# phd3/presto-1

Measured on AMD Instinct MI355X. Metric: probe_rows_per_sec, higher is better.
Workload: dtype int64+f64

## Files before the change

presto-1_amd/csrc/agg.h:

```cpp
#pragma once
#include <cstdlib>

#include "common.h"

namespace tgpu {

constexpr int kLimbs = 68;
constexpr int kMaxAggs = 16;
constexpr int64_t kOrdChainMaxGroups = 65536, kOrdChainMinRows = 256;
constexpr int64_t kOrdHandoffRows = 4096;
inline int64_t ord_chain_max_groups() { const char *e = getenv("TGPU_ORD_CHAIN_MAX_GROUPS"); return e ? atoll(e) : kOrdChainMaxGroups; }

class GroupedAccumulators {
public:
    GroupedAccumulators(Context *ctx, std::vector<tgpu_agg_spec> specs, int32_t step);

    void add_input(const int32_t *gids, int64_t n, const DevicePage &page, int64_t group_count, bool gids_ascending = false);
    void add_intermediate(const int32_t *gids, int64_t n, const DevicePage &page, int64_t group_count, bool gids_ascending = false);
    void evaluate(int64_t group_count, std::vector<DeviceColumn> &out);
    struct DeviceState {
        int32_t function;
        long long *counts;
        long long *limbs;
        unsigned int *special;
        unsigned long long *i128;
        double *dsum;
    };
    void reserve(int64_t groups) { ensure(groups > 0 ? groups : 1); }
    bool begin_ordered(const int32_t *gids, int64_t n, int64_t groups, int64_t lowcard_max_groups, BufferPtr &keys, BufferPtr &rows);
    BufferPtr group_stretches(const unsigned int *keys, int64_t n, int64_t ids);
    void set_allow_ordered(bool on) { allow_ordered_ = on; }
    void set_force_ordered(bool on) { force_ordered_ = on; }
    void set_combine_ordered(bool on) { combine_ordered_ = on; }
    bool force_ordered() const { return force_ordered_ && allow_ordered_; }
    bool ordered() const { return mode_ == Mode::ORDERED; }
    static constexpr int64_t kModePrefixRows = 65536;
    bool decided() const { return mode_ != Mode::UNDECIDED; }
    void decide(int64_t groups_in_prefix, int64_t lowcard_max_groups = 0);
    static int64_t groups_among(Context *ctx, const int32_t *gids, const uint8_t *gids8, int64_t m);
    DeviceState device_state(int k) const;
    struct FoldScratch {
        unsigned long long *partials;
        int32_t stride;
        unsigned long long *pending;
    };
    FoldScratch fold_scratch(int64_t blocks, int64_t group_capacity);
    void flush_fold();
    void resolve_pending(int64_t blocks, bool commit);
    struct HostStates {
        int64_t groups = 0;
        struct Agg {
            std::vector<long long> counts, limbs;
            std::vector<unsigned int> special;
            std::vector<unsigned long long> i128;
            std::vector<double> dsum;
        };
        std::vector<Agg> aggs;
        int64_t bytes() const;
    };
    HostStates dump(int64_t groups);
    void merge(const int32_t *gids, const HostStates &run, int64_t live_groups);
    const std::vector<tgpu_agg_spec> specs() const;
    int output_channel_count() const;
    int intermediate_channel_count() const;
    int64_t estimated_size() const;

private:
    struct State {
        tgpu_agg_spec spec;
        BufferPtr counts;
        BufferPtr limbs;
        BufferPtr special;
        BufferPtr i128;
        BufferPtr dsum;
        int64_t cap = 0;
    };
    enum class Mode { UNDECIDED, EXACT, ORDERED };
    void ensure(int64_t groups);
    void decide_mode(int64_t groups, int64_t lowcard_max_groups);
    void sort_rows_by_group(const int32_t *gids, int64_t n, int64_t groups, BufferPtr &keys, BufferPtr &rows, bool gids_ascending = false);
    Mode mode_ = Mode::UNDECIDED;
    bool allow_ordered_ = false, force_ordered_ = false;
    Context *ctx_;
    std::vector<State> states_;
    int32_t step_;
    BufferPtr error_;
    BufferPtr fold_partials_, fold_pending_;
    bool combine_ordered_ = false;
    int64_t fold_rows_ = 0, fold_stride_ = 0;
    bool fold_dirty_ = false;
};

}
```

presto-1_amd/csrc/agg.hip:

```cpp
#include "agg.h"
#include "kernels.h"
#include "device_agg.h"

#include <rocprim/rocprim.hpp>

#include <algorithm>
#include <cstdlib>

namespace tgpu {

namespace {

constexpr int kBlock = 256;

struct AggView {
    int32_t function;
    int32_t pad;
    const void *input;
    const uint8_t *input_nulls;
    const uint8_t *mask;
    const uint8_t *mask_nulls;
    const void *input2;
    const uint8_t *input2_nulls;
    long long *counts;
    long long *limbs;
    unsigned int *special;
    unsigned long long *i128;
    double *dsum;
};

struct AggArgs {
    int32_t n_aggs;
    int32_t pad;
    AggView a[kMaxAggs];
};

#define kulisch_add tg_kulisch_add
#define i128_add tg_i128_add

template <bool INTERMEDIATE>
__global__ void __launch_bounds__(kBlock) agg_accumulate_kernel(AggArgs args, const int32_t *__restrict__ gids, int64_t n)
{
    for (int64_t r = (int64_t)blockIdx.x * kBlock + threadIdx.x; r < n; r += (int64_t)gridDim.x * kBlock) {
        const int64_t g = gids ? gids[r] : 0;
        if (g < 0) continue;
        for (int k = 0; k < args.n_aggs; k++) {
            const AggView &a = args.a[k];
            if (INTERMEDIATE) {
                const long long cnt = ((const long long *)a.input)[r];
                if (a.function == TGPU_AGG_COUNT_ALL || a.function == TGPU_AGG_COUNT_COLUMN) {
                    if (cnt) atomicAdd((unsigned long long *)&a.counts[g], (unsigned long long)cnt);
                    continue;
                }
                if (cnt == 0) continue;
                atomicAdd((unsigned long long *)&a.counts[g], (unsigned long long)cnt);
                if (a.function == TGPU_AGG_SUM_BIGINT) i128_add(&a.i128[g * 2], ((const long long *)a.input2)[r]);
                else if (tg_is_minmax(a.function)) tg_minmax_update(&a.i128[g * 2], tg_minmax_encode(a.function, ((const unsigned long long *)a.input2)[r]));
                else kulisch_add(&a.limbs[g * kLimbs], &a.special[g], ((const double *)a.input2)[r]);
                continue;
            }
            if (a.mask && ((a.mask_nulls && a.mask_nulls[r]) || !a.mask[r])) continue;
            if (a.function == TGPU_AGG_COUNT_ALL) {
                atomicAdd((unsigned long long *)&a.counts[g], 1ULL);
                continue;
            }
            if (a.input_nulls && a.input_nulls[r]) continue;
            atomicAdd((unsigned long long *)&a.counts[g], 1ULL);
            switch (a.function) {
            case TGPU_AGG_SUM_BIGINT: i128_add(&a.i128[g * 2], ((const long long *)a.input)[r]); break;
            case TGPU_AGG_MIN_BIGINT:
            case TGPU_AGG_MAX_BIGINT:
            case TGPU_AGG_MIN_DOUBLE:
            case TGPU_AGG_MAX_DOUBLE: tg_minmax_update(&a.i128[g * 2], tg_minmax_encode(a.function, ((const unsigned long long *)a.input)[r])); break;
            case TGPU_AGG_SUM_DOUBLE:
            case TGPU_AGG_AVG_DOUBLE: kulisch_add(&a.limbs[g * kLimbs], &a.special[g], ((const double *)a.input)[r]); break;
            case TGPU_AGG_AVG_BIGINT: kulisch_add(&a.limbs[g * kLimbs], &a.special[g], (double)((const long long *)a.input)[r]); break;
            default: break;
            }
        }
    }
}


__global__ void __launch_bounds__(kBlock) ordered_keys_kernel(const int32_t *__restrict__ gids, int64_t n, unsigned int *__restrict__ keys, int *__restrict__ rows,
                                                               unsigned int *__restrict__ unsorted)
{
    bool bad = false;
    for (int64_t r = (int64_t)blockIdx.x * kBlock + threadIdx.x; r < n; r += (int64_t)gridDim.x * kBlock) {
        const int32_t g = gids[r];
        keys[r] = (unsigned int)(g + 1);
        rows[r] = (int)r;
        bad = bad || (r > 0 && gids[r - 1] > g);
    }
    if (unsorted && __any(bad) && (threadIdx.x & 63) == 0) *unsorted = 1u;
}

__global__ void __launch_bounds__(kBlock) ordered_stretches_kernel(const unsigned int *__restrict__ keys, int64_t n, int *__restrict__ stretches)
{
    for (int64_t i = (int64_t)blockIdx.x * kBlock + threadIdx.x; i < n; i += (int64_t)gridDim.x * kBlock) {
        const unsigned int k = keys[i];
        if (k == 0) continue;
        if (i == 0 || keys[i - 1] != k) stretches[(size_t)(k - 1) * 2] = (int)i;
        if (i == n - 1 || keys[i + 1] != k) stretches[(size_t)(k - 1) * 2 + 1] = (int)(i + 1);
    }
}

template <bool INTERMEDIATE>
__global__ void __launch_bounds__(kBlock) agg_ordered_kernel(AggArgs args, const unsigned int *__restrict__ keys, const int *__restrict__ rows, int64_t n,
                                                              unsigned int *error, int64_t handoff, long long *list, unsigned int *list_count)
{
    for (int64_t i = (int64_t)blockIdx.x * kBlock + threadIdx.x; i < n; i += (int64_t)gridDim.x * kBlock) {
        const unsigned int key = keys[i];
        if (key == 0 || (i > 0 && keys[i - 1] == key)) continue;
        const int64_t g = (int64_t)key - 1;
        const int64_t stop = handoff > 0 ? (i + handoff < n ? i + handoff : n) : n;
        if (handoff > 0 && stop < n && keys[stop] == key) {
            const unsigned int at = atomicAdd(list_count, 1u);
            list[(size_t)at * 2] = g;
            list[(size_t)at * 2 + 1] = stop;
        }
#pragma unroll
        for (int k = 0; k < kMaxAggs; k++) {
            if (k >= args.n_aggs) break;
            const AggView &a = args.a[k];
            long long cnt = 0;
            double s = a.dsum ? a.dsum[g] : 0.0;
            __int128 big = 0;
            unsigned long long best = 0;
            for (int64_t j = i; j < stop && keys[j] == key; j++) {
                const int64_t r = rows[j];
                if (INTERMEDIATE) {
                    const long long c = ((const long long *)a.input)[r];
                    if (c == 0) continue;
                    cnt += c;
                    if (a.function == TGPU_AGG_SUM_BIGINT) big += ((const long long *)a.input2)[r];
                    else if (tg_is_minmax(a.function)) {
                        const unsigned long long c_ = tg_minmax_encode(a.function, ((const unsigned long long *)a.input2)[r]);
                        best = c_ > best ? c_ : best;
                    }
                    else if (a.function != TGPU_AGG_COUNT_ALL && a.function != TGPU_AGG_COUNT_COLUMN) s += ((const double *)a.input2)[r];
                    continue;
                }
                if (a.mask && ((a.mask_nulls && a.mask_nulls[r]) || !a.mask[r])) continue;
                if (a.function != TGPU_AGG_COUNT_ALL && a.input_nulls && a.input_nulls[r]) continue;
                cnt++;
                switch (a.function) {
                case TGPU_AGG_SUM_BIGINT: big += ((const long long *)a.input)[r]; break;
                case TGPU_AGG_MIN_BIGINT:
                case TGPU_AGG_MAX_BIGINT:
                case TGPU_AGG_MIN_DOUBLE:
                case TGPU_AGG_MAX_DOUBLE: {
                    const unsigned long long c_ = tg_minmax_encode(a.function, ((const unsigned long long *)a.input)[r]);
                    best = c_ > best ? c_ : best;
                    break;
                }
                case TGPU_AGG_SUM_DOUBLE:
                case TGPU_AGG_AVG_DOUBLE: s += ((const double *)a.input)[r]; break;
                case TGPU_AGG_AVG_BIGINT: s += (double)((const long long *)a.input)[r]; break;
                default: break;
                }
            }
            if (cnt) a.counts[g] += cnt;
            if (a.dsum) a.dsum[g] = s;
            if (best) tg_minmax_update(&a.i128[g * 2], best);
            if (a.i128 && big != 0) {
                const unsigned __int128 cur = ((unsigned __int128)a.i128[g * 2 + 1] << 64) | a.i128[g * 2];
                const unsigned __int128 nxt = cur + (unsigned __int128)big;
                a.i128[g * 2] = (unsigned long long)nxt;
                a.i128[g * 2 + 1] = (unsigned long long)(nxt >> 64);
            }
        }
    }
    (void)error;
}

struct OrdChainPlan {
    int32_t slot[kMaxAggs];
};

__device__ inline long long wave_sum_i64(long long v)
{
#pragma unroll
    for (int d = 32; d >= 1; d >>= 1) v += __shfl_xor(v, d, 64);
    return v;
}

__device__ inline void ordered_chain_group(const AggArgs &args, const OrdChainPlan &plan, const int *__restrict__ rows, int64_t g, long long s, long long e, double *vals,
                                           unsigned long long *cnt_lds, unsigned long long *lo_lds, long long *hi_lds)
{
    const int wave = threadIdx.x >> 6, lane = threadIdx.x & 63;
    if (threadIdx.x < kMaxAggs) {
        cnt_lds[threadIdx.x] = 0;
        lo_lds[threadIdx.x] = 0;
        hi_lds[threadIdx.x] = 0;
    }
    double *sum = nullptr;
    if (wave == 0) {
        __builtin_amdgcn_s_setprio(3);
#pragma unroll
        for (int k = 0; k < kMaxAggs; k++)
            if (k < args.n_aggs && plan.slot[k] == lane) sum = args.a[k].dsum;
    }
    double os = sum ? sum[g] : 0.0;
    __syncthreads();
    const long long tiles = (e - s + TG_ORD_TILE - 1) / TG_ORD_TILE;
    const int r = (wave - 1) * 64 + lane;
    long long row_next = (wave > 0 && s + r < e) ? rows[s + r] : 0;
    for (long long t = 0; t <= tiles; t++) {
        if (wave > 0 && t < tiles) {
            const long long j = s + t * TG_ORD_TILE + r;
            const long long row = row_next;
            if (j + TG_ORD_TILE < e) row_next = rows[j + TG_ORD_TILE];
            double *out = vals + (t & 1) * (TG_ORD_MAX_DOUBLES * TG_ORD_STRIDE) + r;
            const bool live = j < e;
#pragma unroll
            for (int k = 0; k < kMaxAggs; k++) {
                if (k >= args.n_aggs) break;
                const AggView &a = args.a[k];
                bool take = live;
                if (take && a.mask && ((a.mask_nulls && a.mask_nulls[row]) || !a.mask[row])) take = false;
                if (take && a.function != TGPU_AGG_COUNT_ALL && a.input_nulls && a.input_nulls[row]) take = false;
                const unsigned long long taken = __ballot(take);
                if (lane == 0 && taken) atomicAdd(&cnt_lds[k], (unsigned long long)__popcll(taken));
                if (a.function == TGPU_AGG_SUM_BIGINT) {
                    const long long v = take ? ((const long long *)a.input)[row] : 0;
                    const long long lo = wave_sum_i64((long long)(unsigned int)v), hi = wave_sum_i64(v >> 32);
                    if (lane == 0 && taken) {
                        atomicAdd(&lo_lds[k], (unsigned long long)lo);
                        atomicAdd((unsigned long long *)&hi_lds[k], (unsigned long long)hi);
                    }
                }
                else if (tg_is_minmax(a.function)) {
                    if (take) tg_minmax_update(&a.i128[g * 2], tg_minmax_encode(a.function, ((const unsigned long long *)a.input)[row]));
                }
                else if (plan.slot[k] >= 0 && live) {
                    double x = -0.0;
                    if (take) x = a.function == TGPU_AGG_AVG_BIGINT ? (double)((const long long *)a.input)[row] : ((const double *)a.input)[row];
                    out[plan.slot[k] * TG_ORD_STRIDE] = x;
                }
            }
        }
        else if (wave == 0 && t > 0 && sum) {
            const long long left = e - (s + (t - 1) * TG_ORD_TILE);
            os = tg_chain_add_tile(vals + ((t - 1) & 1) * (TG_ORD_MAX_DOUBLES * TG_ORD_STRIDE) + lane * TG_ORD_STRIDE, left < TG_ORD_TILE ? (int)left : TG_ORD_TILE, os);
        }
        __syncthreads();
    }
    if (sum) sum[g] = os;
    if (threadIdx.x == 64) {
#pragma unroll
        for (int k = 0; k < kMaxAggs; k++) {
            if (k >= args.n_aggs) break;
            const AggView &a = args.a[k];
            if (cnt_lds[k]) a.counts[g] += (long long)cnt_lds[k];
            if (a.function == TGPU_AGG_SUM_BIGINT && a.i128) {
                const __int128 big = (__int128)hi_lds[k] * ((__int128)1 << 32) + (__int128)lo_lds[k];
                const unsigned __int128 cur = ((unsigned __int128)a.i128[g * 2 + 1] << 64) | a.i128[g * 2];
                const unsigned __int128 nxt = cur + (unsigned __int128)big;
                a.i128[g * 2] = (unsigned long long)nxt;
                a.i128[g * 2 + 1] = (unsigned long long)(nxt >> 64);
            }
        }
    }
    __syncthreads();
}

__global__ void __launch_bounds__(TG_ORD_WAVES * 64) agg_ordered_chain_kernel(AggArgs args, OrdChainPlan plan, const int *__restrict__ stretches,
                                                                               const unsigned int *__restrict__ keys, const int *__restrict__ rows, int64_t n,
                                                                               const long long *__restrict__ list, const unsigned int *__restrict__ list_count)
{
    __shared__ __attribute__((aligned(16))) double vals[2 * TG_ORD_MAX_DOUBLES * TG_ORD_STRIDE];
    __shared__ unsigned long long cnt_lds[kMaxAggs], lo_lds[kMaxAggs];
    __shared__ long long hi_lds[kMaxAggs];
    if (stretches) {
        const long long s = stretches[(size_t)blockIdx.x * 2], e = stretches[(size_t)blockIdx.x * 2 + 1];
        if (e > s) ordered_chain_group(args, plan, rows, blockIdx.x, s, e, vals, cnt_lds, lo_lds, hi_lds);
        return;
    }
    const unsigned int count = *list_count;
    for (unsigned int b = blockIdx.x; b < count; b += gridDim.x) {
        const long long g = list[(size_t)b * 2], s = list[(size_t)b * 2 + 1];
        long long lo = s, hi = n;
        while (lo < hi) { const long long mid = (lo + hi) >> 1; if (keys[mid] <= (unsigned int)(g + 1)) lo = mid + 1; else hi = mid; }
        if (lo > s) ordered_chain_group(args, plan, rows, g, s, lo, vals, cnt_lds, lo_lds, hi_lds);
    }
}

using LowCardPlan = TgLowCardPlan;

struct LowCardStates {
    TgAggState st[kMaxAggs];
};

__global__ void __launch_bounds__(kBlock) agg_lowcard_kernel(AggArgs args, LowCardStates states, LowCardPlan plan, const int32_t *__restrict__ gids, int64_t n,
                                                              TgFoldScratch fold)
{
    extern __shared__ __attribute__((aligned(16))) unsigned char lds[];
    tg_lc_zero(lds, plan);
    for (int64_t r = (int64_t)blockIdx.x * kBlock + threadIdx.x; r < n; r += (int64_t)gridDim.x * kBlock) {
        const int g = gids ? gids[r] : 0;
        if (g < 0) continue;
        double *hi_base = tg_lc_hi(lds, plan, g), *lo_base = tg_lc_lo(lds, plan, g);
        unsigned int *cnt_base = tg_lc_cnt(lds, plan, g);
        for (int k = 0; k < args.n_aggs; k++) {
            const AggView &a = args.a[k];
            if (a.mask && ((a.mask_nulls && a.mask_nulls[r]) || !a.mask[r])) continue;
            if (a.function != TGPU_AGG_COUNT_ALL && a.input_nulls && a.input_nulls[r]) continue;
            cnt_base[plan.cnt_slot[k] * kBlock + threadIdx.x] += 1u;
            if (tg_is_minmax(a.function)) {
                tg_minmax_update(&a.i128[(size_t)g * 2], tg_minmax_encode(a.function, ((const unsigned long long *)a.input)[r]));
                continue;
            }
            const int w = plan.wide_slot[k];
            if (w < 0) continue;
            if (a.function == TGPU_AGG_SUM_BIGINT) {
                tg_lc_add_bigint(hi_base, lo_base, w, ((const long long *)a.input)[r]);
                continue;
            }
            const double v = a.function == TGPU_AGG_AVG_BIGINT ? (double)((const long long *)a.input)[r] : ((const double *)a.input)[r];
            if (!(fabs(v) <= 1.7976931348623157e308)) {
                tg_flag_special(&a.special[g], v);
                continue;
            }
            const double r = tg_lc_add_double(hi_base, lo_base, w, v);
            if (r != 0.0) tg_kulisch_add(&a.limbs[(size_t)g * kLimbs], &a.special[g], r);
        }
    }
    tg_lc_fold(lds, plan, states.st, fold);
}

__global__ void __launch_bounds__(kBlock) agg_fold_flush_kernel(TgFoldScratch fs, int rows, int n_aggs, LowCardStates states)
{
    tg_fold_flush(fs, rows, n_aggs, states.st);
}

struct KulischWindow {
    int top;
    unsigned int w0, w1, w2;
    bool sticky;
    unsigned int p1, p2;
    bool below;
    __device__ void init() { top = -1; w0 = w1 = w2 = 0; sticky = false; p1 = p2 = 0; below = false; }
    __device__ void push(int i, unsigned int digit)
    {
        if (digit) { top = i; w0 = digit; w1 = p1; w2 = p2; sticky = below; }
        below = below || p2 != 0;
        p2 = p1;
        p1 = digit;
    }
};

__device__ double kulisch_round(const long long *limbs, unsigned int special)
{
    if (special) {
        if ((special & 1u) || ((special & 2u) && (special & 4u))) return __longlong_as_double(0x7ff8000000000000LL);
        return (special & 2u) ? __longlong_as_double(0x7ff0000000000000LL) : __longlong_as_double((long long)0xfff0000000000000ULL);
    }
    KulischWindow pos, negw;
    pos.init();
    negw.init();
    long long carry = 0;
    unsigned int negc = 1;
    for (int i = 0; i < kLimbs; i++) {
        const long long v = limbs[i] + carry;
        const unsigned int digit = (unsigned int)(v & 0xffffffffLL);
        carry = v >> 32;
        pos.push(i, digit);
        const unsigned int nd = ~digit + negc;
        negc = (negc && digit == 0) ? 1u : 0u;
        negw.push(i, nd);
    }
    const bool neg = carry < 0;
    const KulischWindow &w = neg ? negw : pos;
    if (w.top < 0) return 0.0;
    const int hb = 31 - __clz((int)w.w0);
    const int t = w.top * 32 + hb;
    unsigned long long bits;
    if (t <= 52) {
        bits = w.top == 1 ? (((unsigned long long)w.w0 << 32) | w.w1) : (unsigned long long)w.w0;
    }
    else {
        const unsigned __int128 win = ((unsigned __int128)w.w0 << 64) | ((unsigned __int128)w.w1 << 32) | (unsigned __int128)w.w2;
        const int gpos = 64 + hb - 53;
        unsigned long long mant = (unsigned long long)(win >> (gpos + 1));
        const bool guard = (unsigned long long)(win >> gpos) & 1ULL;
        bool sticky = w.sticky || (win & (((unsigned __int128)1 << gpos) - 1)) != 0;
        long long e = (long long)t - 51;
        if (guard && (sticky || (mant & 1ULL))) {
            mant++;
            if (mant >> 53) { mant >>= 1; e++; }
        }
        if (e >= 2047) bits = 0x7ff0000000000000ULL;
        else bits = ((unsigned long long)e << 52) | (mant & 0xfffffffffffffULL);
    }
    if (neg) bits |= 1ULL << 63;
    return __longlong_as_double((long long)bits);
}

struct EvalView {
    int32_t function;
    int32_t partial;
    const long long *counts;
    const long long *limbs;
    const unsigned int *special;
    const unsigned long long *i128;
    const double *dsum;
    void *out0;
    uint8_t *out0_nulls;
    void *out1;
};
struct EvalArgs {
    int32_t n_aggs;
    int32_t pad;
    EvalView a[kMaxAggs];
};

__global__ void __launch_bounds__(kBlock) agg_evaluate_kernel(EvalArgs args, int64_t groups, unsigned int *error)
{
    const int64_t total = groups * args.n_aggs;
    for (int64_t i = (int64_t)blockIdx.x * kBlock + threadIdx.x; i < total; i += (int64_t)gridDim.x * kBlock) {
        const int k = (int)(i % args.n_aggs);
        const int64_t g = i / args.n_aggs;
        const EvalView &a = args.a[k];
        const long long cnt = a.counts[g];
        if (a.function == TGPU_AGG_COUNT_ALL || a.function == TGPU_AGG_COUNT_COLUMN) {
            ((long long *)a.out0)[g] = cnt;
            continue;
        }
        double dsum = 0.0;
        long long lsum = 0;
        if (tg_is_minmax(a.function)) lsum = (long long)tg_minmax_decode(a.function, a.i128[g * 2]);
        else if (a.function == TGPU_AGG_SUM_BIGINT) {
            const unsigned long long lo = a.i128[g * 2], hi = a.i128[g * 2 + 1];
            lsum = (long long)lo;
            const unsigned long long expect_hi = lsum < 0 ? ~0ULL : 0ULL;
            if (hi != expect_hi) atomicOr(error, 1u);
        }
// ... 235 lines not shown
        const HostStates::Agg &r = run.aggs[k];
        MergeArgs::A &a = args.a[k];
        a.function = st.spec.function;
        a.counts = st.counts->as<long long>();
        a.limbs = st.limbs ? st.limbs->as<long long>() : nullptr;
        a.special = st.special ? st.special->as<unsigned int>() : nullptr;
        a.i128 = st.i128 ? st.i128->as<unsigned long long>() : nullptr;
        a.dsum = st.dsum ? st.dsum->as<double>() : nullptr;
        a.r_counts = (const long long *)up(r.counts.data(), r.counts.size() * 8);
        a.r_limbs = (const long long *)up(r.limbs.data(), r.limbs.size() * 8);
        a.r_special = (const unsigned int *)up(r.special.data(), r.special.size() * 4);
        a.r_i128 = (const unsigned long long *)up(r.i128.data(), r.i128.size() * 8);
        a.r_dsum = (const double *)up(r.dsum.data(), r.dsum.size() * 8);
    }
    ctx_->sync();
    ProfileScope ps(ctx_, "agg_merge_states");
    agg_merge_states_kernel<<<grid_for(ctx_, run.groups * kLimbs), kBlock, 0, ctx_->stream()>>>(args, gids, run.groups);
    check_launch("agg_merge_states");
    ctx_->sync();
}

GroupedAccumulators::DeviceState GroupedAccumulators::device_state(int k) const
{
    const State &st = states_[(size_t)k];
    DeviceState d;
    d.function = st.spec.function;
    d.counts = st.counts ? st.counts->as<long long>() : nullptr;
    d.limbs = st.limbs ? st.limbs->as<long long>() : nullptr;
    d.special = st.special ? st.special->as<unsigned int>() : nullptr;
    d.i128 = st.i128 ? st.i128->as<unsigned long long>() : nullptr;
    d.dsum = st.dsum ? st.dsum->as<double>() : nullptr;
    return d;
}

const std::vector<tgpu_agg_spec> GroupedAccumulators::specs() const
{
    std::vector<tgpu_agg_spec> v;
    for (auto &s : states_) v.push_back(s.spec);
    return v;
}

int GroupedAccumulators::output_channel_count() const
{
    return step_ == TGPU_STEP_PARTIAL ? intermediate_channel_count() : (int)states_.size();
}

int GroupedAccumulators::intermediate_channel_count() const
{
    int n = 0;
    for (auto &s : states_) n += is_count(s.spec.function) ? 1 : 2;
    return n;
}

int64_t GroupedAccumulators::estimated_size() const
{
    int64_t s = 0;
    for (auto &st : states_) {
        s += st.cap * 8;
        if (st.limbs) s += st.cap * (kLimbs * 8 + 4);
        if (st.dsum) s += st.cap * 8;
        if (st.i128) s += st.cap * 16;
    }
    return s;
}

void GroupedAccumulators::ensure(int64_t groups)
{
    ZeroList zeros{};
    for (auto &st : states_) {
        if (groups <= st.cap) continue;
        int64_t cap = st.cap ? st.cap : 256;
        while (cap < groups) cap <<= 1;
        st.counts = grow(ctx_, st.counts, st.cap, cap, 8, zeros);
        if (is_double_state(st.spec.function)) {
            if (mode_ == Mode::ORDERED) st.dsum = grow(ctx_, st.dsum, st.cap, cap, 8, zeros);
            else {
                st.limbs = grow(ctx_, st.limbs, st.cap * kLimbs, cap * kLimbs, 8, zeros);
                st.special = grow(ctx_, st.special, st.cap, cap, 4, zeros);
            }
        }
        if (is_bigint_state(st.spec.function)) st.i128 = grow(ctx_, st.i128, st.cap * 2, cap * 2, 8, zeros);
        st.cap = cap;
    }
    if (zeros.n) {
        unsigned long long most = 0;
        for (int i = 0; i < zeros.n; i++) most = std::max(most, zeros.words[i]);
        multi_zero_kernel<<<grid_for(ctx_, (int64_t)most), kBlock, 0, ctx_->stream()>>>(zeros);
        check_launch("multi_zero");
    }
}

static void check_channel(const DevicePage &page, int ch, int32_t want_type, const char *what)
{
    TG_CHECK_ARG(ch >= 0 && ch < (int)page.cols.size(), std::string(what) + ": channel out of range");
    if (want_type) TG_CHECK_ARG(page.cols[ch].type == want_type, std::string(what) + ": unexpected channel type " + type_name(page.cols[ch].type));
}

static int64_t lowcard_bytes_per_group(const std::vector<tgpu_agg_spec> &specs)
{
    int64_t wide = 0;
    for (auto &s : specs) wide += (is_count(s.function) || is_minmax(s.function)) ? 0 : 1;
    return wide * 2 * kBlock * 8 + (int64_t)specs.size() * kBlock * 4;
}

void GroupedAccumulators::decide_mode(int64_t groups, int64_t lowcard_max_groups)
{
    if (mode_ != Mode::UNDECIDED) return;
    const bool many = groups > lowcard_max_groups || force_ordered_;
    mode_ = (allow_ordered_ && many && getenv("TGPU_DISABLE_ORDERED") == nullptr) ? Mode::ORDERED : Mode::EXACT;
}

void GroupedAccumulators::decide(int64_t groups_in_prefix, int64_t lowcard_max_groups)
{
    if (lowcard_max_groups <= 0) lowcard_max_groups = (160 * 1024) / std::max<int64_t>(lowcard_bytes_per_group(specs()), 1);
    decide_mode(groups_in_prefix > 0 ? groups_in_prefix : 1, lowcard_max_groups);
}

static __global__ void __launch_bounds__(kBlock) max_gid_kernel(const int32_t *__restrict__ gids, const uint8_t *__restrict__ gids8, int64_t m, int *out)
{
    int best = -1;
    for (int64_t i = (int64_t)blockIdx.x * kBlock + threadIdx.x; i < m; i += (int64_t)gridDim.x * kBlock) {
        const int g = gids8 ? (int)gids8[i] - 1 : gids[i];
        best = g > best ? g : best;
    }
#pragma unroll
    for (int d = 32; d >= 1; d >>= 1) {
        const int o = __shfl_down(best, d, 64);
        best = o > best ? o : best;
    }
    if ((threadIdx.x & 63) == 0 && best >= 0) atomicMax(out, best);
}

int64_t GroupedAccumulators::groups_among(Context *ctx, const int32_t *gids, const uint8_t *gids8, int64_t m)
{
    if (m <= 0 || (!gids && !gids8)) return 0;
    BufferPtr out = ctx->alloc(4);
    HIP_CHECK(hipMemsetAsync(out->ptr(), 0xff, 4, ctx->stream()));
    max_gid_kernel<<<(int)std::min<int64_t>(ceil_div(m, kBlock), 64), kBlock, 0, ctx->stream()>>>(gids, gids8, m, out->as<int>());
    check_launch("max_gid");
    return (int64_t)ctx->read_scalar(out->as<int>()) + 1;
}

bool GroupedAccumulators::begin_ordered(const int32_t *gids, int64_t n, int64_t groups, int64_t lowcard_max_groups, BufferPtr &keys, BufferPtr &rows)
{
    if (n <= 0) return false;
    decide_mode(groups > 0 ? groups : 1, lowcard_max_groups);
    if (mode_ != Mode::ORDERED) return false;
    TG_CHECK_STATE(gids != nullptr, "ordered accumulation needs int32 group ids");
    ensure(groups > 0 ? groups : 1);
    sort_rows_by_group(gids, n, groups, keys, rows);
    return true;
}

BufferPtr GroupedAccumulators::group_stretches(const unsigned int *keys, int64_t n, int64_t ids)
{
    BufferPtr st = ctx_->alloc_zero((size_t)ids * 8);
    ordered_stretches_kernel<<<grid_for(ctx_, n), kBlock, 0, ctx_->stream()>>>(keys, n, st->as<int>());
    check_launch("ordered_stretches");
    return st;
}

void GroupedAccumulators::sort_rows_by_group(const int32_t *gids, int64_t n, int64_t groups, BufferPtr &keys, BufferPtr &rows, bool gids_ascending)
{
    const bool always_sort = getenv("TGPU_ALWAYS_SORT") != nullptr;
    const bool known = gids_ascending && !always_sort;
    BufferPtr keys_in = ctx_->alloc((size_t)n * 4), rows_in = ctx_->alloc((size_t)n * 4), unsorted = known ? nullptr : ctx_->alloc_zero(4);
    ordered_keys_kernel<<<grid_for(ctx_, n), kBlock, 0, ctx_->stream()>>>(gids, n, keys_in->as<unsigned int>(), rows_in->as<int>(),
                                                                          known ? nullptr : unsorted->as<unsigned int>());
    check_launch("ordered_keys");
    if (known || (!always_sort && ctx_->read_scalar(unsorted->as<unsigned int>()) == 0)) {
        keys = keys_in;
        rows = rows_in;
        return;
    }
    keys = ctx_->alloc((size_t)n * 4);
    rows = ctx_->alloc((size_t)n * 4);
    unsigned int end_bit = 1;
    while (end_bit < 32 && (1ull << end_bit) <= (unsigned long long)groups) end_bit++;
    size_t temp_bytes = 0;
    HIP_CHECK(rocprim::radix_sort_pairs(nullptr, temp_bytes, keys_in->as<unsigned int>(), keys->as<unsigned int>(), rows_in->as<int>(), rows->as<int>(), (size_t)n, 0,
                                        end_bit, ctx_->stream()));
    BufferPtr temp = ctx_->alloc(temp_bytes ? temp_bytes : 1);
    HIP_CHECK(rocprim::radix_sort_pairs(temp->ptr(), temp_bytes, keys_in->as<unsigned int>(), keys->as<unsigned int>(), rows_in->as<int>(), rows->as<int>(), (size_t)n, 0,
                                        end_bit, ctx_->stream()));
}

void GroupedAccumulators::add_input(const int32_t *gids, int64_t n, const DevicePage &page, int64_t group_count, bool gids_ascending)
{
    if (states_.empty() || n <= 0) return;
    BufferPtr zero_gids;
    if (!gids && force_ordered()) {
        zero_gids = ctx_->alloc_zero((size_t)n * 4);
        gids = zero_gids->as<int32_t>();
    }
    if (gids) decide_mode(group_count > 0 ? group_count : 1, (160 * 1024) / std::max<int64_t>(lowcard_bytes_per_group(specs()), 1));
    else if (mode_ == Mode::UNDECIDED) mode_ = Mode::EXACT;
    {
        const int64_t lowcard_capacity = (160 * 1024) / std::max<int64_t>(lowcard_bytes_per_group(specs()), 1);
        const int64_t g = group_count > 0 ? group_count : 1;
        ensure(mode_ == Mode::EXACT && g <= lowcard_capacity ? lowcard_capacity : g);
    }
    AggArgs args{};
    args.n_aggs = (int32_t)states_.size();
    for (size_t k = 0; k < states_.size(); k++) {
        State &st = states_[k];
        AggView &a = args.a[k];
        a.function = st.spec.function;
        if (st.spec.function != TGPU_AGG_COUNT_ALL) {
            int32_t want = 0;
            if (bigint_valued(st.spec.function) || st.spec.function == TGPU_AGG_AVG_BIGINT) want = TGPU_BIGINT;
            if (st.spec.function == TGPU_AGG_MIN_DOUBLE || st.spec.function == TGPU_AGG_MAX_DOUBLE) want = TGPU_DOUBLE;
            if (st.spec.function == TGPU_AGG_SUM_DOUBLE || st.spec.function == TGPU_AGG_AVG_DOUBLE) want = TGPU_DOUBLE;
            check_channel(page, st.spec.input_channel, want, "aggregate input");
            a.input = page.cols[st.spec.input_channel].values;
            a.input_nulls = page.cols[st.spec.input_channel].nulls;
        }
        if (st.spec.mask_channel >= 0) {
            check_channel(page, st.spec.mask_channel, TGPU_BOOLEAN, "aggregate mask");
            a.mask = (const uint8_t *)page.cols[st.spec.mask_channel].values;
            a.mask_nulls = page.cols[st.spec.mask_channel].nulls;
        }
        a.counts = st.counts->as<long long>();
        a.limbs = st.limbs ? st.limbs->as<long long>() : nullptr;
        a.special = st.special ? st.special->as<unsigned int>() : nullptr;
        a.i128 = st.i128 ? st.i128->as<unsigned long long>() : nullptr;
        a.dsum = st.dsum ? st.dsum->as<double>() : nullptr;
    }
    if (mode_ == Mode::ORDERED) {
        TG_CHECK_STATE(gids != nullptr, "ordered accumulation needs group ids");
        OrdChainPlan plan{};
        int doubles = 0;
        for (int k = 0; k < kMaxAggs; k++) plan.slot[k] = (k < args.n_aggs && args.a[k].dsum) ? doubles++ : -1;
        const int64_t ids = group_count > 0 ? group_count : 1;
        const bool chained = doubles <= TG_ORD_MAX_DOUBLES && ids <= ord_chain_max_groups() && n >= ids * kOrdChainMinRows && getenv("TGPU_DISABLE_ORDERED_CHAIN") == nullptr;
        BufferPtr keys, rows;
        const int64_t long_groups = n / kOrdHandoffRows;
        const bool handoff = !chained && long_groups > 0 && doubles <= TG_ORD_MAX_DOUBLES && getenv("TGPU_DISABLE_ORDERED_CHAIN") == nullptr;
        BufferPtr list, list_count;
        {
            ProfileScope ps(ctx_, chained ? "agg_accumulate_ordered_chain" : "agg_accumulate_ordered");
            sort_rows_by_group(gids, n, group_count, keys, rows, gids_ascending);
            if (chained) {
                BufferPtr stretches = group_stretches(keys->as<unsigned int>(), n, ids);
                agg_ordered_chain_kernel<<<(int)ids, TG_ORD_WAVES * 64, 0, ctx_->stream()>>>(args, plan, stretches->as<int>(), keys->as<unsigned int>(), rows->as<int>(), n,
                                                                                              nullptr, nullptr);
                check_launch("agg_accumulate_ordered_chain");
                return;
            }
            if (handoff) {
                list = ctx_->alloc((size_t)long_groups * 16);
                list_count = ctx_->alloc_zero(8);
            }
            agg_ordered_kernel<false><<<grid_for(ctx_, n), kBlock, 0, ctx_->stream()>>>(args, keys->as<unsigned int>(), rows->as<int>(), n, error_->as<unsigned int>(),
                                                                                          handoff ? kOrdHandoffRows : 0, handoff ? list->as<long long>() : nullptr,
                                                                                          handoff ? list_count->as<unsigned int>() : nullptr);
            check_launch("agg_accumulate_ordered");
        }
        if (handoff) {
            ProfileScope ps(ctx_, "agg_accumulate_ordered_handoff");
            agg_ordered_chain_kernel<<<(int)std::min<int64_t>(long_groups, ctx_->cu_count()), TG_ORD_WAVES * 64, 0, ctx_->stream()>>>(
                args, plan, nullptr, keys->as<unsigned int>(), rows->as<int>(), n, list->as<long long>(), list_count->as<unsigned int>());
            check_launch("agg_accumulate_ordered_handoff");
        }
        return;
    }
    LowCardPlan plan{};
    plan.n_aggs = args.n_aggs;
    for (int k = 0; k < args.n_aggs; k++) {
        plan.wide_slot[k] = (is_count(args.a[k].function) || is_minmax(args.a[k].function)) ? -1 : plan.n_wide++;
        plan.cnt_slot[k] = k;
        plan.count_from_rows[k] = 0;
    }
    plan.n_cnt = plan.n_aggs;
    plan.rows_slot = -1;
    plan.per_group_bytes = plan.n_wide * 2 * kBlock * 8 + plan.n_cnt * kBlock * 4;
    const int64_t groups = group_count > 0 ? group_count : 1;
    const int64_t lds_bytes = groups * plan.per_group_bytes;
    const bool lowcard_enabled = getenv("TGPU_DISABLE_LOWCARD") == nullptr;
    if (lowcard_enabled && lds_bytes <= 160 * 1024 && n >= 4096) {
        plan.n_groups = (int32_t)groups;
        static bool attr_set = false;
        if (!attr_set) {
            HIP_CHECK(hipFuncSetAttribute((const void *)agg_lowcard_kernel, hipFuncAttributeMaxDynamicSharedMemorySize, 160 * 1024));
            attr_set = true;
        }
        const int per_cu = (int)std::max<int64_t>(1, std::min<int64_t>(8, (160 * 1024) / lds_bytes));
        int64_t blocks = std::min<int64_t>((int64_t)ctx_->cu_count() * per_cu, ceil_div(n, kBlock));
        ProfileScope ps(ctx_, "agg_accumulate_lowcard");
        LowCardStates states{};
        for (int k = 0; k < args.n_aggs; k++) {
            states.st[k].function = args.a[k].function;
            states.st[k].counts = args.a[k].counts;
            states.st[k].limbs = args.a[k].limbs;
            states.st[k].special = args.a[k].special;
            states.st[k].i128 = args.a[k].i128;
            states.st[k].dsum = nullptr;
        }
        const FoldScratch fs = fold_scratch(blocks, (160 * 1024) / plan.per_group_bytes);
        agg_lowcard_kernel<<<(int)blocks, kBlock, (size_t)lds_bytes, ctx_->stream()>>>(args, states, plan, gids, n, TgFoldScratch{fs.partials, fs.stride, nullptr});
        check_launch("agg_accumulate_lowcard");
        return;
    }
    ProfileScope ps(ctx_, "agg_accumulate");
    agg_accumulate_kernel<false><<<grid_for(ctx_, n), kBlock, 0, ctx_->stream()>>>(args, gids, n);
    check_launch("agg_accumulate");
}

void GroupedAccumulators::add_intermediate(const int32_t *gids, int64_t n, const DevicePage &page, int64_t group_count, bool gids_ascending)
{
    if (states_.empty() || n <= 0) return;
    BufferPtr zero_gids;
    if (!gids && force_ordered()) {
        zero_gids = ctx_->alloc_zero((size_t)n * 4);
        gids = zero_gids->as<int32_t>();
    }
    if (gids) decide_mode(group_count > 0 ? group_count : 1, (160 * 1024) / std::max<int64_t>(lowcard_bytes_per_group(specs()), 1));
    else if (mode_ == Mode::UNDECIDED) mode_ = Mode::EXACT;
    ensure(group_count > 0 ? group_count : 1);
    AggArgs args{};
    args.n_aggs = (int32_t)states_.size();
    for (size_t k = 0; k < states_.size(); k++) {
        State &st = states_[k];
        AggView &a = args.a[k];
        a.function = st.spec.function;
        int ch = st.spec.input_channel;
        check_channel(page, ch, TGPU_BIGINT, "intermediate count");
        a.input = page.cols[ch].values;
        ch++;
        if (!is_count(st.spec.function)) {
            check_channel(page, ch, bigint_valued(st.spec.function) ? TGPU_BIGINT : TGPU_DOUBLE, "intermediate sum");
            a.input2 = page.cols[ch].values;
            ch++;
        }
        a.counts = st.counts->as<long long>();
        a.limbs = st.limbs ? st.limbs->as<long long>() : nullptr;
        a.special = st.special ? st.special->as<unsigned int>() : nullptr;
        a.i128 = st.i128 ? st.i128->as<unsigned long long>() : nullptr;
        a.dsum = st.dsum ? st.dsum->as<double>() : nullptr;
    }
    if (mode_ == Mode::ORDERED) {
        TG_CHECK_STATE(gids != nullptr, "ordered accumulation needs group ids");
        ProfileScope ps(ctx_, "agg_combine_ordered");
        BufferPtr keys, rows;
        sort_rows_by_group(gids, n, group_count, keys, rows, gids_ascending && zero_gids == nullptr);
        agg_ordered_kernel<true><<<grid_for(ctx_, n), kBlock, 0, ctx_->stream()>>>(args, keys->as<unsigned int>(), rows->as<int>(), n, error_->as<unsigned int>(), 0, nullptr,
                                                                                     nullptr);
        check_launch("agg_combine_ordered");
        return;
    }
    ProfileScope ps(ctx_, "agg_combine");
    agg_accumulate_kernel<true><<<grid_for(ctx_, n), kBlock, 0, ctx_->stream()>>>(args, gids, n);
    check_launch("agg_combine");
}

void GroupedAccumulators::evaluate(int64_t groups, std::vector<DeviceColumn> &out)
{
    if (states_.empty()) return;
    ensure(groups > 0 ? groups : 1);
    flush_fold();
    EvalArgs args{};
    args.n_aggs = (int32_t)states_.size();
    const bool partial = step_ == TGPU_STEP_PARTIAL;
    const int64_t alloc_n = groups > 0 ? groups : 1;
    for (size_t k = 0; k < states_.size(); k++) {
        State &st = states_[k];
        EvalView &a = args.a[k];
        a.function = st.spec.function;
        a.partial = partial ? 1 : 0;
        a.counts = st.counts->as<long long>();
        a.limbs = st.limbs ? st.limbs->as<long long>() : nullptr;
        a.special = st.special ? st.special->as<unsigned int>() : nullptr;
        a.i128 = st.i128 ? st.i128->as<unsigned long long>() : nullptr;
        a.dsum = st.dsum ? st.dsum->as<double>() : nullptr;
        DeviceColumn c0;
        c0.n = groups;
        c0.values_buf = ctx_->alloc((size_t)alloc_n * 8);
        c0.values = c0.values_buf->ptr();
        a.out0 = c0.values_buf->ptr();
        if (is_count(st.spec.function) || partial) {
            c0.type = TGPU_BIGINT;
            out.push_back(c0);
            if (partial && !is_count(st.spec.function)) {
                DeviceColumn c1;
                c1.n = groups;
                c1.type = bigint_valued(st.spec.function) ? TGPU_BIGINT : TGPU_DOUBLE;
                c1.values_buf = ctx_->alloc((size_t)alloc_n * 8);
                c1.values = c1.values_buf->ptr();
                a.out1 = c1.values_buf->ptr();
                out.push_back(c1);
            }
        }
        else {
            c0.type = bigint_valued(st.spec.function) ? TGPU_BIGINT : TGPU_DOUBLE;
            c0.nulls_buf = ctx_->alloc((size_t)alloc_n);
            c0.nulls = c0.nulls_buf->as<uint8_t>();
            a.out0_nulls = c0.nulls_buf->as<uint8_t>();
            out.push_back(c0);
        }
    }
    if (groups <= 0) return;
    HIP_CHECK(hipMemsetAsync(error_->ptr(), 0, 4, ctx_->stream()));
    {
        ProfileScope ps(ctx_, "agg_evaluate");
        agg_evaluate_kernel<<<grid_for(ctx_, groups * args.n_aggs), kBlock, 0, ctx_->stream()>>>(args, groups, error_->as<unsigned int>());
        check_launch("agg_evaluate");
    }
    bool can_raise = false;
    for (auto &st : states_) can_raise = can_raise || st.spec.function == TGPU_AGG_SUM_BIGINT;
    if (can_raise) {
        unsigned int err = ctx_->read_scalar(error_->as<unsigned int>());
        if (err) fail(TGPU_ERR_NUMERIC_VALUE_OUT_OF_RANGE, "bigint addition overflow");
    }
}

// ... 2 lines not shown
```

Before: 92.19 billion.

## Skip group sort for ascending gids and add tiled run-based ordered aggregation kernel

When group ids already arrive in ascending order, the ordered aggregation path skips building sorted key/row arrays and reads gids directly through an abstraction used by the stretch, chain and handoff kernels. For the non-chained case it adds a new kernel that stages each tile's values and take-masks in LDS, finds run heads via ballot, and has one thread walk each run, extending past the tile edge and handing very long runs to the chain kernel. This removes the sort/key-materialisation pass and the indirect row gathers. The cost is larger dynamic LDS use per block and serial per-run walks, which may lower occupancy or load-balance poorly when runs are long.

```diff
diff --git a/presto-1_amd/csrc/agg.h b/presto-1_amd/csrc/agg.h
--- a/presto-1_amd/csrc/agg.h
+++ b/presto-1_amd/csrc/agg.h
@@ -28,7 +28,7 @@
     };
     void reserve(int64_t groups) { ensure(groups > 0 ? groups : 1); }
     bool begin_ordered(const int32_t *gids, int64_t n, int64_t groups, int64_t lowcard_max_groups, BufferPtr &keys, BufferPtr &rows);
-    BufferPtr group_stretches(const unsigned int *keys, int64_t n, int64_t ids);
+    BufferPtr group_stretches(const unsigned int *keys, int64_t n, int64_t ids, const int32_t *ascending_gids = nullptr);
     void set_allow_ordered(bool on) { allow_ordered_ = on; }
     void set_force_ordered(bool on) { force_ordered_ = on; }
     void set_combine_ordered(bool on) { combine_ordered_ = on; }
diff --git a/presto-1_amd/csrc/agg.hip b/presto-1_amd/csrc/agg.hip
--- a/presto-1_amd/csrc/agg.hip
+++ b/presto-1_amd/csrc/agg.hip
@@ -95,13 +95,21 @@
     if (unsorted && __any(bad) && (threadIdx.x & 63) == 0) *unsorted = 1u;
 }
 
-__global__ void __launch_bounds__(kBlock) ordered_stretches_kernel(const unsigned int *__restrict__ keys, int64_t n, int *__restrict__ stretches)
+struct OrdOrder {
+    const unsigned int *keys;
+    const int *rows;
+    const int32_t *gids;
+    __device__ __forceinline__ unsigned int key(int64_t i) const { return keys ? keys[i] : (unsigned int)(gids[i] + 1); }
+    __device__ __forceinline__ int64_t row(int64_t i) const { return keys ? (int64_t)rows[i] : i; }
+};
+
+__global__ void __launch_bounds__(kBlock) ordered_stretches_kernel(OrdOrder ord, int64_t n, int *__restrict__ stretches)
 {
     for (int64_t i = (int64_t)blockIdx.x * kBlock + threadIdx.x; i < n; i += (int64_t)gridDim.x * kBlock) {
-        const unsigned int k = keys[i];
+        const unsigned int k = ord.key(i);
         if (k == 0) continue;
-        if (i == 0 || keys[i - 1] != k) stretches[(size_t)(k - 1) * 2] = (int)i;
-        if (i == n - 1 || keys[i + 1] != k) stretches[(size_t)(k - 1) * 2 + 1] = (int)(i + 1);
+        if (i == 0 || ord.key(i - 1) != k) stretches[(size_t)(k - 1) * 2] = (int)i;
+        if (i == n - 1 || ord.key(i + 1) != k) stretches[(size_t)(k - 1) * 2 + 1] = (int)(i + 1);
     }
 }
 
@@ -185,7 +193,7 @@
     return v;
 }
 
-__device__ inline void ordered_chain_group(const AggArgs &args, const OrdChainPlan &plan, const int *__restrict__ rows, int64_t g, long long s, long long e, double *vals,
+__device__ inline void ordered_chain_group(const AggArgs &args, const OrdChainPlan &plan, const OrdOrder &ord, int64_t g, long long s, long long e, double *vals,
                                            unsigned long long *cnt_lds, unsigned long long *lo_lds, long long *hi_lds)
 {
     const int wave = threadIdx.x >> 6, lane = threadIdx.x & 63;
@@ -205,12 +213,12 @@
     __syncthreads();
     const long long tiles = (e - s + TG_ORD_TILE - 1) / TG_ORD_TILE;
     const int r = (wave - 1) * 64 + lane;
-    long long row_next = (wave > 0 && s + r < e) ? rows[s + r] : 0;
+    long long row_next = (wave > 0 && s + r < e) ? ord.row(s + r) : 0;
     for (long long t = 0; t <= tiles; t++) {
         if (wave > 0 && t < tiles) {
             const long long j = s + t * TG_ORD_TILE + r;
             const long long row = row_next;
-            if (j + TG_ORD_TILE < e) row_next = rows[j + TG_ORD_TILE];
+            if (j + TG_ORD_TILE < e) row_next = ord.row(j + TG_ORD_TILE);
             double *out = vals + (t & 1) * (TG_ORD_MAX_DOUBLES * TG_ORD_STRIDE) + r;
             const bool live = j < e;
 #pragma unroll
@@ -265,8 +273,7 @@
     __syncthreads();
 }
 
-__global__ void __launch_bounds__(TG_ORD_WAVES * 64) agg_ordered_chain_kernel(AggArgs args, OrdChainPlan plan, const int *__restrict__ stretches,
-                                                                               const unsigned int *__restrict__ keys, const int *__restrict__ rows, int64_t n,
+__global__ void __launch_bounds__(TG_ORD_WAVES * 64) agg_ordered_chain_kernel(AggArgs args, OrdChainPlan plan, const int *__restrict__ stretches, OrdOrder ord, int64_t n,
                                                                                const long long *__restrict__ list, const unsigned int *__restrict__ list_count)
 {
     __shared__ __attribute__((aligned(16))) double vals[2 * TG_ORD_MAX_DOUBLES * TG_ORD_STRIDE];
@@ -274,15 +281,206 @@
     __shared__ long long hi_lds[kMaxAggs];
     if (stretches) {
         const long long s = stretches[(size_t)blockIdx.x * 2], e = stretches[(size_t)blockIdx.x * 2 + 1];
-        if (e > s) ordered_chain_group(args, plan, rows, blockIdx.x, s, e, vals, cnt_lds, lo_lds, hi_lds);
+        if (e > s) ordered_chain_group(args, plan, ord, blockIdx.x, s, e, vals, cnt_lds, lo_lds, hi_lds);
         return;
     }
     const unsigned int count = *list_count;
     for (unsigned int b = blockIdx.x; b < count; b += gridDim.x) {
         const long long g = list[(size_t)b * 2], s = list[(size_t)b * 2 + 1];
         long long lo = s, hi = n;
-        while (lo < hi) { const long long mid = (lo + hi) >> 1; if (keys[mid] <= (unsigned int)(g + 1)) lo = mid + 1; else hi = mid; }
-        if (lo > s) ordered_chain_group(args, plan, rows, g, s, lo, vals, cnt_lds, lo_lds, hi_lds);
+        while (lo < hi) { const long long mid = (lo + hi) >> 1; if (ord.key(mid) <= (unsigned int)(g + 1)) lo = mid + 1; else hi = mid; }
+        if (lo > s) ordered_chain_group(args, plan, ord, g, s, lo, vals, cnt_lds, lo_lds, hi_lds);
+    }
+}
+
+constexpr int kOrdRunIters = 8, kOrdRunTile = kBlock * kOrdRunIters, kOrdRunStaged = 3, kOrdRunChunk = 8;
+constexpr size_t kOrdRunFixedLds = 64 + 2 * (size_t)(kOrdRunTile + 8) * 2 + (size_t)kOrdRunTile * 4 + 32 * 4;
+static_assert(kOrdHandoffRows >= kOrdRunTile, "a walk that is handed over ends beyond its tile");
+
+struct OrdRunPlan {
+    int32_t slot[kMaxAggs];
+    int32_t staged, pad;
+};
+
+__device__ __forceinline__ unsigned long long ord_run_addend(int function, unsigned long long raw, bool take)
+{
+    switch (function) {
+    case TGPU_AGG_SUM_BIGINT: return take ? raw : 0ULL;
+    case TGPU_AGG_MIN_BIGINT:
+    case TGPU_AGG_MAX_BIGINT:
+    case TGPU_AGG_MIN_DOUBLE:
+    case TGPU_AGG_MAX_DOUBLE: return take ? tg_minmax_encode(function, raw) : 0ULL;
+    case TGPU_AGG_AVG_BIGINT: return take ? (unsigned long long)__double_as_longlong((double)(long long)raw) : 0x8000000000000000ULL;
+    default: return take ? raw : 0x8000000000000000ULL;
+    }
+}
+
+enum { kOrdCount = 0, kOrdDouble = 1, kOrdBig = 2, kOrdMinMax = 3 };
+
+template <int KIND>
+__device__ __forceinline__ void ord_run_walk(const unsigned long long *v, const unsigned short *cnt_lds, int k, int j, int e, int &cnt, double &s, __int128 &big,
+                                             unsigned long long &best)
+{
+    for (int jj = j; jj < e; jj += kOrdRunChunk) {
+        unsigned short c[kOrdRunChunk];
+        unsigned long long x[kOrdRunChunk];
+#pragma unroll
+        for (int u = 0; u < kOrdRunChunk; u++) {
+            c[u] = cnt_lds[jj + u];
+            x[u] = KIND == kOrdCount ? 0ULL : v[jj + u];
+        }
+#pragma unroll
+        for (int u = 0; u < kOrdRunChunk; u++) {
+            const bool in = jj + u < e;
+            cnt += in ? (c[u] >> k) & 1 : 0;
+            if (KIND == kOrdDouble) s = in ? s + __longlong_as_double((long long)x[u]) : s;
+            if (KIND == kOrdBig) big += in ? (long long)x[u] : 0LL;
+            if (KIND == kOrdMinMax) best = (in && x[u] > best) ? x[u] : best;
+        }
+    }
+}
+
+__global__ void __launch_bounds__(kBlock) agg_ordered_runs_kernel(AggArgs args, OrdRunPlan plan, const int32_t *__restrict__ gids, int64_t n, int64_t handoff,
+                                                                   long long *list, unsigned int *list_count)
+{
+    extern __shared__ __attribute__((aligned(16))) unsigned char lds[];
+    unsigned long long *val_lds = (unsigned long long *)lds;
+    unsigned short *cnt_lds = (unsigned short *)(lds + (size_t)plan.staged * kOrdRunTile * 8 + 64);
+    unsigned short *head_lds = cnt_lds + kOrdRunTile + 8;
+    int32_t *gid_lds = (int32_t *)(head_lds + kOrdRunTile + 8);
+    int *wave_lds = (int *)(gid_lds + kOrdRunTile);
+    const int wave = threadIdx.x >> 6, lane = threadIdx.x & 63;
+    const int64_t tiles = (n + kOrdRunTile - 1) / kOrdRunTile;
+    for (int64_t t = blockIdx.x; t < tiles; t += gridDim.x) {
+        const int64_t base = t * kOrdRunTile;
+        const int m = (int)(n - base < kOrdRunTile ? n - base : kOrdRunTile);
+        int32_t gid[kOrdRunIters], before[kOrdRunIters];
+        unsigned int counted[kOrdRunIters];
+        int64_t row[kOrdRunIters];
+#pragma unroll
+        for (int it = 0; it < kOrdRunIters; it++) {
+            const int j = it * kBlock + threadIdx.x;
+            row[it] = base + (j < m ? j : m - 1);
+            gid[it] = gids[row[it]];
+            before[it] = gids[row[it] > 0 ? row[it] - 1 : 0];
+            counted[it] = 0;
+        }
+#pragma unroll
+        for (int k = 0; k < kMaxAggs; k++) {
+            if (k >= args.n_aggs) break;
+            const AggView &a = args.a[k];
+            const int slot = plan.slot[k];
+            unsigned long long raw[kOrdRunIters];
+            uint8_t mk[kOrdRunIters], mkn[kOrdRunIters], inn[kOrdRunIters];
+#pragma unroll
+            for (int it = 0; it < kOrdRunIters; it++) {
+                raw[it] = 0ULL;
+                mk[it] = 1;
+                mkn[it] = 0;
+                inn[it] = 0;
+            }
+            if (slot >= 0) {
+#pragma unroll
+                for (int it = 0; it < kOrdRunIters; it++) raw[it] = ((const unsigned long long *)a.input)[row[it]];
+            }
+            if (a.mask) {
+#pragma unroll
+                for (int it = 0; it < kOrdRunIters; it++) mk[it] = a.mask[row[it]];
+            }
+            if (a.mask && a.mask_nulls) {
+#pragma unroll
+                for (int it = 0; it < kOrdRunIters; it++) mkn[it] = a.mask_nulls[row[it]];
+            }
+            if (a.function != TGPU_AGG_COUNT_ALL && a.input_nulls) {
+#pragma unroll
+                for (int it = 0; it < kOrdRunIters; it++) inn[it] = a.input_nulls[row[it]];
+            }
+#pragma unroll
+            for (int it = 0; it < kOrdRunIters; it++) {
+                const bool take = (mk[it] != 0) & (mkn[it] == 0) & (inn[it] == 0);
+                counted[it] |= (take ? 1u : 0u) << k;
+                if (slot >= 0) val_lds[(size_t)slot * kOrdRunTile + it * kBlock + threadIdx.x] = ord_run_addend(a.function, raw[it], take);
+            }
+        }
+        int rank[kOrdRunIters];
+#pragma unroll
+        for (int it = 0; it < kOrdRunIters; it++) {
+            const int j = it * kBlock + threadIdx.x;
+            cnt_lds[j] = (unsigned short)counted[it];
+            gid_lds[j] = gid[it];
+            const bool head = j < m && (base + j == 0 || before[it] != gid[it]);
+            const unsigned long long heads = __ballot(head);
+            rank[it] = head ? __popcll(heads & ((1ULL << lane) - 1ULL)) : -1;
+            if (lane == 0) wave_lds[it * (kBlock / 64) + wave] = __popcll(heads);
+        }
+        __syncthreads();
+        int runs = 0;
+#pragma unroll
+        for (int w = 0; w < kOrdRunIters * (kBlock / 64); w++) {
+            if ((w & 3) == wave) {
+                const int it = w >> 2;
+                if (rank[it] >= 0) head_lds[runs + rank[it]] = (unsigned short)(it * kBlock + threadIdx.x);
+            }
+            runs += wave_lds[w];
+        }
+        if (threadIdx.x == 0) head_lds[runs] = (unsigned short)m;
+        __syncthreads();
+        for (int h = threadIdx.x; h < runs; h += kBlock) {
+            const int j = head_lds[h], e = head_lds[h + 1];
+            const int32_t g32 = gid_lds[j];
+            const int64_t g = g32, i = base + j;
+            double start[kMaxAggs];
+#pragma unroll
+            for (int k = 0; k < kMaxAggs; k++) {
+                start[k] = 0.0;
+                if (k < args.n_aggs && args.a[k].dsum) start[k] = args.a[k].dsum[g];
+            }
+            const int64_t stop = handoff > 0 ? (i + handoff < n ? i + handoff : n) : n;
+            int64_t ge = base + e;
+            if (e == m)
+                while (ge < stop && gids[ge] == g32) ge++;
+            if (handoff > 0 && ge == stop && stop < n && gids[stop] == g32) {
+                const unsigned int at = atomicAdd(list_count, 1u);
+                list[(size_t)at * 2] = g;
+                list[(size_t)at * 2 + 1] = stop;
+            }
+#pragma unroll
+            for (int k = 0; k < kMaxAggs; k++) {
+                if (k >= args.n_aggs) break;
+                const AggView &a = args.a[k];
+                const int slot = plan.slot[k];
+                const unsigned long long *v = val_lds + (size_t)(slot >= 0 ? slot : 0) * kOrdRunTile;
+                int c = 0;
+                double s = start[k];
+                __int128 big = 0;
+                unsigned long long best = 0;
+                if (slot < 0) ord_run_walk<kOrdCount>(v, cnt_lds, k, j, e, c, s, big, best);
+                else if (a.function == TGPU_AGG_SUM_BIGINT) ord_run_walk<kOrdBig>(v, cnt_lds, k, j, e, c, s, big, best);
+                else if (tg_is_minmax(a.function)) ord_run_walk<kOrdMinMax>(v, cnt_lds, k, j, e, c, s, big, best);
+                else ord_run_walk<kOrdDouble>(v, cnt_lds, k, j, e, c, s, big, best);
+                long long cnt = c;
+                for (int64_t r = base + e; r < ge; r++) {
+                    if (a.mask && ((a.mask_nulls && a.mask_nulls[r]) || !a.mask[r])) continue;
+                    if (a.function != TGPU_AGG_COUNT_ALL && a.input_nulls && a.input_nulls[r]) continue;
+                    cnt++;
+                    if (slot < 0) continue;
+                    const unsigned long long x = ord_run_addend(a.function, ((const unsigned long long *)a.input)[r], true);
+                    if (a.function == TGPU_AGG_SUM_BIGINT) big += (long long)x;
+                    else if (tg_is_minmax(a.function)) best = x > best ? x : best;
+                    else s += __longlong_as_double((long long)x);
+                }
+                if (cnt) atomicAdd((unsigned long long *)&a.counts[g], (unsigned long long)cnt);
+                if (a.dsum) a.dsum[g] = s;
+                if (best) tg_minmax_update(&a.i128[g * 2], best);
+                if (a.i128 && big != 0) {
+                    const unsigned __int128 cur = ((unsigned __int128)a.i128[g * 2 + 1] << 64) | a.i128[g * 2];
+                    const unsigned __int128 nxt = cur + (unsigned __int128)big;
+                    a.i128[g * 2] = (unsigned long long)nxt;
+                    a.i128[g * 2 + 1] = (unsigned long long)(nxt >> 64);
+                }
+            }
+        }
+        __syncthreads();
     }
 }
 
@@ -824,10 +1022,10 @@
     return true;
 }
 
-BufferPtr GroupedAccumulators::group_stretches(const unsigned int *keys, int64_t n, int64_t ids)
+BufferPtr GroupedAccumulators::group_stretches(const unsigned int *keys, int64_t n, int64_t ids, const int32_t *ascending_gids)
 {
     BufferPtr st = ctx_->alloc_zero((size_t)ids * 8);
-    ordered_stretches_kernel<<<grid_for(ctx_, n), kBlock, 0, ctx_->stream()>>>(keys, n, st->as<int>());
+    ordered_stretches_kernel<<<grid_for(ctx_, n), kBlock, 0, ctx_->stream()>>>(OrdOrder{keys, nullptr, ascending_gids}, n, st->as<int>());
     check_launch("ordered_stretches");
     return st;
 }
@@ -909,13 +1107,21 @@
         const int64_t long_groups = n / kOrdHandoffRows;
         const bool handoff = !chained && long_groups > 0 && doubles <= TG_ORD_MAX_DOUBLES && getenv("TGPU_DISABLE_ORDERED_CHAIN") == nullptr;
         BufferPtr list, list_count;
+        OrdRunPlan run_plan{};
+        for (int k = 0; k < kMaxAggs; k++) run_plan.slot[k] = (k < args.n_aggs && !is_count(args.a[k].function)) ? run_plan.staged++ : -1;
+        const char *run_switch = getenv("TGPU_AGG_RUN_ORDERED");
+        const bool list_free = gids_ascending && getenv("TGPU_ALWAYS_SORT") == nullptr && !(run_switch && atoi(run_switch) == 0) &&
+                               (chained || run_plan.staged <= kOrdRunStaged);
+        OrdOrder ord{nullptr, nullptr, gids};
         {
             ProfileScope ps(ctx_, chained ? "agg_accumulate_ordered_chain" : "agg_accumulate_ordered");
-            sort_rows_by_group(gids, n, group_count, keys, rows, gids_ascending);
+            if (!list_free) {
+                sort_rows_by_group(gids, n, group_count, keys, rows, gids_ascending);
+                ord = OrdOrder{keys->as<unsigned int>(), rows->as<int>(), gids};
+            }
             if (chained) {
-                BufferPtr stretches = group_stretches(keys->as<unsigned int>(), n, ids);
-                agg_ordered_chain_kernel<<<(int)ids, TG_ORD_WAVES * 64, 0, ctx_->stream()>>>(args, plan, stretches->as<int>(), keys->as<unsigned int>(), rows->as<int>(), n,
-                                                                                              nullptr, nullptr);
+                BufferPtr stretches = group_stretches(ord.keys, n, ids, gids);
+                agg_ordered_chain_kernel<<<(int)ids, TG_ORD_WAVES * 64, 0, ctx_->stream()>>>(args, plan, stretches->as<int>(), ord, n, nullptr, nullptr);
                 check_launch("agg_accumulate_ordered_chain");
                 return;
             }
@@ -923,15 +1129,30 @@
                 list = ctx_->alloc((size_t)long_groups * 16);
                 list_count = ctx_->alloc_zero(8);
             }
-            agg_ordered_kernel<false><<<grid_for(ctx_, n), kBlock, 0, ctx_->stream()>>>(args, keys->as<unsigned int>(), rows->as<int>(), n, error_->as<unsigned int>(),
-                                                                                          handoff ? kOrdHandoffRows : 0, handoff ? list->as<long long>() : nullptr,
-                                                                                          handoff ? list_count->as<unsigned int>() : nullptr);
+            if (list_free) {
+                const size_t lds_bytes = (size_t)run_plan.staged * kOrdRunTile * 8 + kOrdRunFixedLds;
+                static bool attr_set = false;
+                if (!attr_set) {
+                    HIP_CHECK(hipFuncSetAttribute((const void *)agg_ordered_runs_kernel, hipFuncAttributeMaxDynamicSharedMemorySize,
+                                                  (int)((size_t)kOrdRunStaged * kOrdRunTile * 8 + kOrdRunFixedLds)));
+                    attr_set = true;
+                }
+                int64_t blocks = grid_for(ctx_, n, kOrdRunTile);
+                if (const char *cap = getenv("TGPU_AGG_RUN_MAX_BLOCKS")) blocks = std::max<int64_t>(1, std::min<int64_t>(blocks, atoll(cap)));
+                agg_ordered_runs_kernel<<<(int)blocks, kBlock, lds_bytes, ctx_->stream()>>>(args, run_plan, gids, n, handoff ? kOrdHandoffRows : 0,
+                                                                                           handoff ? list->as<long long>() : nullptr,
+                                                                                           handoff ? list_count->as<unsigned int>() : nullptr);
+            }
+            else
+                agg_ordered_kernel<false><<<grid_for(ctx_, n), kBlock, 0, ctx_->stream()>>>(args, ord.keys, ord.rows, n, error_->as<unsigned int>(),
+                                                                                              handoff ? kOrdHandoffRows : 0, handoff ? list->as<long long>() : nullptr,
+                                                                                              handoff ? list_count->as<unsigned int>() : nullptr);
             check_launch("agg_accumulate_ordered");
         }
         if (handoff) {
             ProfileScope ps(ctx_, "agg_accumulate_ordered_handoff");
             agg_ordered_chain_kernel<<<(int)std::min<int64_t>(long_groups, ctx_->cu_count()), TG_ORD_WAVES * 64, 0, ctx_->stream()>>>(
-                args, plan, nullptr, keys->as<unsigned int>(), rows->as<int>(), n, list->as<long long>(), list_count->as<unsigned int>());
+                args, plan, nullptr, ord, n, list->as<long long>(), list_count->as<unsigned int>());
             check_launch("agg_accumulate_ordered_handoff");
         }
         return;
```

After: 94.15 billion (median of 6 runs). 1.02x the previous value.
